# olsson-group/thermodynamic-interpolation

Hardware: AMD Instinct MI355X
Metric: integration-steps/sec (whole node) + drift rel-L2 vs CPU ref (higher is better)
Workload: dtype f32 state and accumulation; matrix products on fp16 MFMA with 2-way split fp32 operands (hi + lo halves, 3 products)

## Files before the change

### thermodynamic-interpolation_amd/csrc/api_painn.hip

```cpp
#include "rollout.hpp"

extern "C" {

ti_handle* ti_painn_create(const ti_painn_desc* d, const float* weights, size_t n_weights, const int32_t* edge_src,
                           const int32_t* edge_dst, const int32_t* edge_type, const int32_t* atom_ids, int device)
{
    ti_handle* out = nullptr;
    const int rc = guarded([&]() -> int {
        if (!d || !weights || !atom_ids) return fail(TI_E_ARG, "NULL argument");
        const int F = d->n_features, L = d->n_layers, A = d->n_atoms, E = d->n_edges;
        if (F != 32 && F != 64 && F != 128 && F != 256) return fail(TI_E_UNSUPPORTED, "n_features must be 32, 64, 128 or 256");
        if (L < 1) return fail(TI_E_ARG, "n_layers must be >= 1");
        if (A < 1 || A > 32) return fail(TI_E_UNSUPPORTED, "n_atoms must be in 1..32 (the reference caps it at n_types = 25)");
        if (E < 0 || (E > 0 && (!edge_src || !edge_dst || !edge_type))) return fail(TI_E_ARG, "edge arrays missing");
        if (d->variant < 0 || d->variant > 2) return fail(TI_E_ARG, "unknown variant");
        if (d->n_types < 1) return fail(TI_E_ARG, "n_types must be >= 1");
        if (d->precision != TI_PREC_F32 && d->precision != TI_PREC_F16X2 && d->precision != TI_PREC_F16) return fail(TI_E_ARG, "unknown precision");
        for (int k = 0; k < E; ++k)
            if (edge_src[k] < 0 || edge_src[k] >= A || edge_dst[k] < 0 || edge_dst[k] >= A || edge_type[k] < 0 || edge_type[k] > 3)
                return fail(TI_E_ARG, "edge index / type out of range");
        for (int a = 0; a < A; ++a) if (atom_ids[a] < 0 || atom_ids[a] >= d->n_types) return fail(TI_E_ARG, "atom id out of range");
        std::unique_ptr<ti_handle> h(new_handle(0, device));
        h->d = *d; h->NB = F / 32;
        h->nE = d->variant == TI_VARIANT_AMBIENT ? 4 : d->variant == TI_VARIANT_LATENT_MULTI ? 3 : 2;
// ... 223 lines not shown
            if (n_floats != N * F) return fail(TI_E_ARG, "size mismatch (s)");
            std::vector<float> ds(n_floats);
            HIP_CHECK(hipMemcpy(out, h->s.p, n_floats * sizeof(float), hipMemcpyDeviceToHost));
            HIP_CHECK(hipMemcpy(ds.data(), h->dsacc.p, n_floats * sizeof(float), hipMemcpyDeviceToHost));
            for (size_t i = 0; i < n_floats; ++i) out[i] += ds[i];
        } else if (what == 1) {
            if (n_floats != N * 3 * F) return fail(TI_E_ARG, "size mismatch (v)");
            std::vector<float> v(n_floats), dv(n_floats), cc(n_floats);
            HIP_CHECK(hipMemcpy(v.data(), h->v.p, n_floats * sizeof(float), hipMemcpyDeviceToHost));
            HIP_CHECK(hipMemcpy(dv.data(), h->dvacc.p, n_floats * sizeof(float), hipMemcpyDeviceToHost));
            HIP_CHECK(hipMemcpy(cc.data(), h->cacc.p, n_floats * sizeof(float), hipMemcpyDeviceToHost));
            for (size_t nd = 0; nd < N; ++nd)
                for (size_t f = 0; f < F; ++f)
                    for (int c = 0; c < 3; ++c) {
                        const int c1 = (c + 1) % 3, c2 = (c + 2) % 3;
                        auto at = [&](const std::vector<float>& a, int cc2) { return a[(nd * 3 + cc2) * F + f]; };
                        out[(nd * 3 + c) * F + f] = (at(v, c) + at(dv, c)) + (at(cc, c1) * at(v, c2) - at(cc, c2) * at(v, c1));
                    }
        } else if (what == 2) {
            if (n_floats != B * E * F) return fail(TI_E_ARG, "size mismatch (e)");
            const size_t RB = ti::EDGE_ROWS_PER_BLOCK, rows = (B + h->G - 1) / h->G * h->parts * h->nblk * RB * (h->active == 2 ? 2 : 1);
            std::vector<float> e(rows * F);
            HIP_CHECK(hipMemcpy(e.data(), h->e.p, e.size() * sizeof(float), hipMemcpyDeviceToHost));
            for (size_t m = 0; m < B; ++m)
                for (size_t k = 0; k < E; ++k)
                    std::memcpy(out + (m * E + h->perm[k]) * F, e.data() + edge_row_of(h, m, k) * F, F * sizeof(float));
        } else if (what >= 3 && what <= 5) {
            if (h->last_D != 1 || (size_t)h->last_VB != B) return fail(TI_E_ARG, "tangent taps need a preceding ti_painn_drift_jvp call");
            auto fetch = [&](const DevBuf<float>& b, size_t n) { std::vector<float> v(n); HIP_CHECK(hipMemcpy(v.data(), b.p, n * sizeof(float), hipMemcpyDeviceToHost)); return v; };
            if (what == 3) {
                if (n_floats != N * F) return fail(TI_E_ARG, "size mismatch (ts)");
                const auto ts = fetch(h->ts, n_floats), td = fetch(h->tdsacc, n_floats);
                for (size_t i = 0; i < n_floats; ++i) out[i] = ts[i] + td[i];
            } else if (what == 4) {
                if (n_floats != N * 3 * F) return fail(TI_E_ARG, "size mismatch (tv)");
                const auto v = fetch(h->v, n_floats), cc = fetch(h->cacc, n_floats);
                const auto tv = fetch(h->tv, n_floats), tdv = fetch(h->tdvacc, n_floats), tcc = fetch(h->tcacc, n_floats);
                for (size_t nd = 0; nd < N; ++nd)
                    for (size_t f = 0; f < F; ++f)
                        for (int c = 0; c < 3; ++c) {
                            const int c1 = (c + 1) % 3, c2 = (c + 2) % 3;
                            auto at = [&](const std::vector<float>& a, int cc2) { return a[(nd * 3 + cc2) * F + f]; };
                            out[(nd * 3 + c) * F + f] = (at(tv, c) + at(tdv, c)) + ((at(tcc, c1) * at(v, c2) + at(cc, c1) * at(tv, c2)) -
                                                                                     (at(tcc, c2) * at(v, c1) + at(cc, c2) * at(tv, c1)));
                        }
            } else {
                if (n_floats != B * E * F) return fail(TI_E_ARG, "size mismatch (te)");
                const size_t RB = ti::EDGE_ROWS_PER_BLOCK, rows = (B + h->G - 1) / h->G * h->parts * h->nblk * RB;
                const auto e = fetch(h->te, rows * F);
                for (size_t m = 0; m < B; ++m)
                    for (size_t k = 0; k < E; ++k)
                        std::memcpy(out + (m * E + h->perm[k]) * F, e.data() + edge_row_of(h, m, k) * F, F * sizeof(float));
            }
        } else return fail(TI_E_ARG, "unknown tap");
        return TI_OK;
    });
}

int ti_painn_set_template(ti_handle* h, int which)
{
    if (!h || h->kind != 0) return fail(TI_E_ARG, "not a painn handle");
    if (which != TI_TEMPLATE_AUTO && which != TI_TEMPLATE_THROUGHPUT && which != TI_TEMPLATE_LATENCY && which != TI_TEMPLATE_PAIR) return fail(TI_E_ARG, "unknown template");
    if (which == TI_TEMPLATE_LATENCY && h->n_tpl < 2) which = TI_TEMPLATE_THROUGHPUT;
    if (which == TI_TEMPLATE_PAIR && !h->has_pair) which = TI_TEMPLATE_THROUGHPUT;
    h->pinned_tpl = which;
    return TI_OK;
}

int ti_painn_template_for(ti_handle* h, int64_t B)
{
    if (!h || h->kind != 0) return fail(TI_E_ARG, "not a painn handle");
    if (h->has_pair && mask_blocks_pair(h) && pinned_template(h) == TI_TEMPLATE_PAIR)
        return fail(TI_E_UNSUPPORTED, "the pair layout is pinned, and the edge mask in force is not symmetric for every molecule");
    return template_for(h, B);
}

int ti_painn_set_edge_mask(ti_handle* h, const uint32_t* mask, int64_t B, int mem)
{
    if (mem != TI_MEM_HOST && mem != TI_MEM_DEVICE) return fail(TI_E_ARG, "unknown mem");
    if (mask && B < 1) return fail(TI_E_ARG, "B < 1");
    if (!h || h->kind != 0) return fail(TI_E_ARG, "not a painn handle");
    if (!mask) { clear_graph_state(h); return TI_OK; }
    return guarded([&]() -> int {
        set_device(h);
        const int A = h->d.n_atoms;
        std::vector<uint32_t> m((size_t)B * A);
        if (mem == TI_MEM_DEVICE) HIP_CHECK(hipMemcpy(m.data(), mask, m.size() * sizeof(uint32_t), hipMemcpyDeviceToHost));
        else std::memcpy(m.data(), mask, m.size() * sizeof(uint32_t));
        std::vector<int32_t> none; std::vector<uint8_t> no_types;
        return set_graph_state(h, m, none, no_types, B);
    });
}

int ti_painn_set_molecules(ti_handle* h, const int32_t* n_atoms, const uint32_t* mask, const uint8_t* pair_type, int64_t B, int mem)
{
    if (mem != TI_MEM_HOST && mem != TI_MEM_DEVICE) return fail(TI_E_ARG, "unknown mem");
    if (n_atoms && B < 1) return fail(TI_E_ARG, "B < 1");
    if (!h || h->kind != 0) return fail(TI_E_ARG, "not a painn handle");
    if (!n_atoms) { clear_graph_state(h); return TI_OK; }
    return guarded([&]() -> int {
        set_device(h);
        const int A = h->d.n_atoms;
        auto fetch = [&](void* dst, const void* src, size_t bytes) {
            if (mem == TI_MEM_DEVICE) HIP_CHECK(hipMemcpy(dst, src, bytes, hipMemcpyDeviceToHost));
            else std::memcpy(dst, src, bytes);
        };
// ... 18 lines not shown
```

### thermodynamic-interpolation_amd/csrc/painn_host.hip

```cpp
#include "ti_handle.hpp"

namespace ti {

void ensure_painn_ws(ti_handle* h, long long B)
{
    if (B <= h->cap) return;
    const size_t A = h->d.n_atoms, F = h->d.n_features, N = (size_t)B * A;
    h->x.alloc(N * 3); h->b1.alloc(N * 3); h->b2.alloc(N * 3); h->xt.alloc(N * 3);
    h->cond.alloc(std::max<size_t>(N * h->ncond, 1));
    const size_t se = h->d.precision == TI_PREC_F16 ? 2 : 1;
    h->s.alloc((N * F + se - 1) / se); h->P.alloc((N * F + se - 1) / se);
    h->v.alloc((N * 3 * F + se - 1) / se); h->dvacc.alloc(N * 3 * F); h->cacc.alloc(N * 3 * F); h->dsacc.alloc(N * F);
    h->e.alloc((edge_rows_for(h, B) * F + se - 1) / se);
    h->enc.alloc((edge_rows_for(h, B) * F + se - 1) / se); h->geo.alloc(edge_rows_for(h, B) * 4);
    h->divb.alloc(B); h->div2.alloc(B); h->dl.alloc(B); h->dlscaled.alloc(B);
    h->cap = B;
}

long long jvp_virtual_molecules(const ti_handle* h, long long B, int D) { return (B + h->G - 1) / h->G * D * h->G; }

size_t jvp_bytes_per_vm(const ti_handle* h)
{
    const size_t A = h->d.n_atoms, F = h->d.n_features;
    const size_t erows = ((size_t)h->parts * h->nblk * ti::EDGE_ROWS_PER_BLOCK + h->G - 1) / h->G;
// ... 158 lines not shown
        }
        if (h->nblk > 0) {
            EdgeParams p{};
            p.stream = h->S(h->st_edge[l]); p.nch = h->st_edge[l].nch; p.vecs = h->edge_vecs.p + (size_t)l * 21 * F;
            p.edge_emb = h->F(h->edge_emb); p.rows = h->rows.p; p.slotnode = h->slotnode.p; p.nslots = nullptr;
            p.nblk = h->nblk; p.G = h->G; p.parts = h->parts; p.A = A; p.max_slots = h->max_slots; p.B = B; p.n_groups = groups; p.length_scale = h->d.length_scale;
            p.x = x_dev; p.P = h->P.p; p.v = h->v.p; p.dsacc = h->dsacc.p; p.dvacc = h->dvacc.p; p.cacc = h->cacc.p; p.e = h->e.p; p.enc = h->enc.p; p.geo = h->geo.p;
            for (int i = 0; i < 6; ++i) p.wscale[i] = 1.0f;
            if (edge_one_chain(prec)) {
                p.stream = h->S(h->st_edge1[l]); p.nch = h->st_edge1[l].nch; p.vecs = h->edge_vecs1.p + (size_t)l * 21 * F;
                for (int i = 0; i < 6; ++i) p.wscale[i] = h->edge_scale[(size_t)l * 6 + i];
            }
            if (mrows) p.rows = mrows;
            Timed tm(h, TI_KERNEL_PAINN_EDGE);
#ifdef TI_STAMPS
            if (l == 2) p.stamps = stamps_arm(groups, st);
#endif
            if (h->active == 2) {
                HIP_CHECK(launch_pair(NB, l == 0, l == L - 1, prec, p, st, mrows != nullptr));
#ifdef TI_STAMPS
                stamps_dump(h, p.stamps, groups, st);
#endif
            } else {
                HIP_CHECK(launch_edge(NB, l == 0, l == L - 1, prec, p, st, mrows != nullptr));
#ifdef TI_STAMPS
                stamps_dump(h, p.stamps, groups, st);
#endif
            }
        }
        if (h->tap == 1 + 2 * l) return;
        if (jr) {
            {
                JvpNodeParams p{};
                p.stream = h->S(h->st_jvp_update[l]); p.nch = h->st_jvp_update[l].nch; p.vecs = h->upd_vecs.p + (size_t)l * 10 * F;
                p.N = N; p.s = h->s.p; p.v = h->v.p; p.dsacc = h->dsacc.p; p.dvacc = h->dvacc.p; p.cacc = h->cacc.p;
                p.ns = reinterpret_cast<float4*>(h->nodest.p);
                Timed tm(h, TI_KERNEL_PAINN_JVP_FILTER);
                HIP_CHECK(launch_jvp_node(NB, split, p, st));
            }
            JvpUpdateParams p{};
            p.stream = h->S(h->st_jvp_update[l]); p.nch = h->st_jvp_update[l].nch; p.vecs = h->upd_vecs.p + (size_t)l * 10 * F;
            p.N = VN; p.B = B; p.A = A; p.D = jr->D; p.G = h->G; p.has_next = l + 1 < L;
            p.v = h->v.p; p.cacc = h->cacc.p; p.ns = reinterpret_cast<const float4*>(h->nodest.p);
            p.ts = h->ts.p; p.tv = h->tv.p; p.tdsacc = h->tdsacc.p; p.tdvacc = h->tdvacc.p; p.tcacc = h->tcacc.p; p.tP = h->tP.p;
            p.zero_acc = !ft;
            Timed tm(h, TI_KERNEL_PAINN_JVP_UPDATE);
            HIP_CHECK(launch_jvp_update(NB, split, p, st));
        }
        {
            UpdateParams p{};
            p.stream = h->S(h->st_update[l]); p.nch = h->st_update[l].nch; p.vecs = h->upd_vecs.p + (size_t)l * 10 * F;
            p.N = N; p.s = h->s.p; p.v = h->v.p; p.dsacc = h->dsacc.p; p.dvacc = h->dvacc.p; p.cacc = h->cacc.p; p.P = h->P.p;
            p.first_layer = l == 0; p.zero_acc = !ft;
            const bool folded = h->nblk > 0 && h->active == 2 && l > 0 && pair_folds_cross(prec);
            Timed tm(h, TI_KERNEL_PAINN_UPDATE);
            HIP_CHECK(launch_update(NB, l + 1 < L, prec, p, st, folded));
        }
        if (h->tap == 2 + 2 * l) return;
    }
    if (jr) {
        JvpReadoutParams p{};
        p.stream = h->S(h->st_jvp_readout); p.nch = h->st_jvp_readout.nch; p.vecs = h->jvp_ro_vecs.p; p.b2_gate = h->b2_gate;
        p.N = VN; p.B = B; p.A = A; p.D = jr->D; p.G = h->G; p.s = h->s.p; p.v = h->v.p; p.ts = h->ts.p; p.tv = h->tv.p; p.tout = jr->tout;
        Timed tm(h, TI_KERNEL_PAINN_JVP_READOUT);
        HIP_CHECK(launch_jvp_readout(NB, split, p, st));
    }
    {
        ReadoutParams p{};
        p.stream = h->S(h->st_jvp_readout); p.nch = h->st_jvp_readout.nch; p.mlp = h->vec(h->readout);
        p.w2_gate = h->F(h->readout.W2 + F); p.b2_gate = h->b2_gate; p.Vr = h->F(h->Vr);
        p.N = N; p.s = h->s.p; p.v = h->v.p; p.out = out_dev;
        Timed tm(h, TI_KERNEL_PAINN_READOUT);
        HIP_CHECK(launch_readout(NB, prec, p, st));
    }
    if (nat) {
        HIP_CHECK(launch_zero_pads(out_dev, nat, B, 1, A, 3, st));
        if (jr && jr->D == 1) HIP_CHECK(launch_zero_pads(jr->tout, nat, B, 1, A, 3, st));
    }
}

void painn_drift_div_dev(ti_handle* h, const float* x_dev, float t, const float* cond_dev, long long B, float* out_dev, float* div_dev,
                         const float* tv)
{
    const int A = h->d.n_atoms, D = 3 * A;
    const long long chunk = jvp_chunk_molecules(h, D);
    for (long long b0 = 0; b0 < B; b0 += chunk) {
        const long long bc = std::min(chunk, B - b0);
        ensure_jvp_ws(h, bc, D);
        JvpRun jr{D, nullptr, h->tout.p};
        painn_drift_dev(h, x_dev + (size_t)b0 * A * 3, t, cond_dev ? cond_dev + (size_t)b0 * A * h->ncond : nullptr, bc,
                        out_dev + (size_t)b0 * A * 3, &jr, tv ? tv + b0 : nullptr, b0);
        if (h->ragged) HIP_CHECK(launch_div_reduce_ragged(h->tout.p, bc, D, h->G, h->natoms_dev.p + b0, div_dev + b0, h->stream));
        else HIP_CHECK(launch_div_reduce(h->tout.p, bc, D, h->G, div_dev + b0, h->stream));
    }
    h->last_B = std::min(chunk, B);
}

void painn_make_probes(ti_handle* h, long long B, int k, uint64_t seed, long long traj0)
{
    const int n3 = 3 * h->d.n_atoms;
    grow(h->probes, (size_t)B * k * n3);
    HIP_CHECK(launch_probes(h->probes.p, seed, traj0, B, k, n3, h->stream));
    if (h->ragged) HIP_CHECK(launch_zero_pads(h->probes.p, h->natoms_dev.p, B * k, k, h->d.n_atoms, 3, h->stream));
}

void painn_drift_div_est_dev(ti_handle* h, const float* x_dev, float t, const float* cond_dev, long long B, int k, float* out_dev,
// ... 57 lines not shown
```

### thermodynamic-interpolation_amd/csrc/painn_kernels.hip

```cpp
#include <hip/amd_detail/amd_hip_unsafe_atomics.h>

#include "dispatch.hpp"
#include "mfma_chain.hpp"
#include "ti_internal.hpp"

namespace ti {


struct UV {
    static constexpr int B0 = 0, G0 = 1, BE0 = 2, B1 = 3, G1 = 4, BE1 = 5, B2 = 6 , PB0 = 9, COUNT = 10;
};

__host__ __device__ constexpr int update_superchunk(int NB, bool H16) { return H16 && NB == 4 ? 4 : 2; }
__host__ __device__ constexpr int update_chunk4(int NB, bool H16) { return (H16 ? 128 : 256) * NB; }
template <int NBK, bool HAS_NEXT, int PREC, bool FOLDED = false>
__global__ __launch_bounds__(256, (NBK <= 8 ? 2 : 1)) void painn_update_kernel(const UpdateParams p)
{
    constexpr bool H16 = PREC == 2;
    constexpr int F = 16 * NBK, NB = (F + 31) / 32, WAVES = 4, T = 64 * WAVES, CH4 = update_chunk4(NB, H16);
    using A16 = r16::Act<NBK>;
    using OP = typename r16::OpSel<NBK, PREC>::type;
    extern __shared__ f32x4 lds[];
    const int lane = threadIdx.x & 63, wave = __builtin_amdgcn_readfirstlane(threadIdx.x >> 6), j = lane & 15, q = lane >> 4;
    constexpr int SC = update_superchunk(NB, H16);
    float* vec = reinterpret_cast<float*>(lds + 2 * SC * CH4);
    for (int i = threadIdx.x; i < UV::COUNT * F / 4; i += T)
        reinterpret_cast<f32x4*>(vec)[i] = reinterpret_cast<const f32x4*>(p.vecs)[i];
    PipeDMA<NB, T, SC, CH4> pipe;
    pipe.init(reinterpret_cast<const f32x4*>(p.stream), p.nch, lds, wave, lane);

    const long long node = ((long long)blockIdx.x * WAVES + wave) * 16 + j;
    const bool ok = node < p.N;
    const size_t nd = (size_t)(ok ? node : p.N - 1);
    const size_t vo = nd * 3 * F, so_ = nd * F;
    float* db = p.dvacc + nd * 3 * F;
    float* cb = p.cacc + nd * 3 * F;
    float* ab = p.dsacc + nd * F;

    A16 n2;
    {
        OP ve[3];
        float vsc[3];
        {
            A16 t[3];
#pragma unroll
            for (int nb = 0; nb < NBK; ++nb) {
                f32x4 vv[3], kk[3];
#pragma unroll
                for (int c = 0; c < 3; ++c) {
                    vv[c] = p.first_layer ? f32x4{0, 0, 0, 0} : r16::load_state<H16>(p.v, vo + c * F, nb, q);
                    kk[c] = p.first_layer || FOLDED ? f32x4{0, 0, 0, 0} : r16::load_block(cb + c * F, nb, q);
                }
#pragma unroll
                for (int c = 0; c < 3; ++c) {
                    const int c1 = (c + 1) % 3, c2 = (c + 2) % 3;
                    const f32x4 dd = r16::load_block(db + c * F, nb, q);
                    if (FOLDED) t[c].b[nb] = vv[c] + dd;
                    else t[c].b[nb] = (vv[c] + dd) + (kk[c1] * vv[c2] - kk[c2] * vv[c1]);
                    if (ok) r16::store_block(db + c * F, nb, q, t[c].b[nb]);
                }
            }
#pragma unroll
            for (int c = 0; c < 3; ++c) vsc[c] = ve[c].set_scaled(t[c]);
        }
#pragma unroll
        for (int nb = 0; nb < NBK; ++nb) n2.b[nb] = f32x4{0, 0, 0, 0};
#pragma unroll
        for (int ch = 0; ch < NB; ++ch) {
            const f32x4* wl = pipe.acquire();
#pragma unroll
            for (int c = 0; c < 3; ++c) {
                f32x4 a0 = {0, 0, 0, 0}, a1 = {0, 0, 0, 0};
                r16::gemm_bt(a0, a1, ve[c], wl, lane);
                a0 *= vsc[c]; a1 *= vsc[c];
                n2.b[2 * ch] += a0 * a0; n2.b[2 * ch + 1] += a1 * a1;
            }
            pipe.release();
        }
    }
    A16 snew;
    OP h2;
    {
        A16 t;
#pragma unroll
        for (int nb = 0; nb < NBK; ++nb) t.b[nb] = r16::load_block(vec + UV::B0 * F, nb, q);
        {
            OP nn;
            float nsc;
            {
                A16 u;
#pragma unroll
                for (int nb = 0; nb < NBK; ++nb)
#pragma unroll
                    for (int r = 0; r < 4; ++r) u.b[nb][r] = sqrtf(n2.b[nb][r]);
                nsc = nn.set_scaled(u);
            }
#pragma unroll
            for (int ch = 0; ch < NB; ++ch) {
                const f32x4* wl = pipe.acquire();
                f32x4 g0 = {0, 0, 0, 0}, g1 = {0, 0, 0, 0};
                r16::gemm_bt(g0, g1, nn, wl, lane);
                t.b[2 * ch] += g0 * nsc; t.b[2 * ch + 1] += g1 * nsc;
                pipe.release();
            }
        }
        {
            OP ss;
            float ssc;
#pragma unroll
            for (int nb = 0; nb < NBK; ++nb) snew.b[nb] = r16::load_state<H16>(p.s, so_, nb, q) + r16::load_block(ab, nb, q);
            ssc = ss.set_scaled(snew);
#pragma unroll
// ... 5 lines not shown
                pipe.release();
            }
        }
        r16::ln_silu(t, vec + UV::G0 * F, vec + UV::BE0 * F, q);
        OP h1;
        h1.set(t);
#pragma unroll
        for (int ch = 0; ch < NB; ++ch) {
            const f32x4* wl = pipe.acquire();
            f32x4 a0 = r16::load_block(vec + UV::B1 * F, 2 * ch, q), a1 = r16::load_block(vec + UV::B1 * F, 2 * ch + 1, q);
            r16::gemm_bt(a0, a1, h1, wl, lane);
            t.b[2 * ch] = a0; t.b[2 * ch + 1] = a1;
            pipe.release();
        }
        r16::ln_silu(t, vec + UV::G1 * F, vec + UV::BE1 * F, q);
        h2.set(t);
    }
#pragma unroll
    for (int ch = 0; ch < NB; ++ch) {
        const f32x4* wl = pipe.acquire();
        f32x4 q0 = r16::load_block(vec + (UV::B2 + 1) * F, 2 * ch, q), q1 = r16::load_block(vec + (UV::B2 + 1) * F, 2 * ch + 1, q);
        r16::gemm_bt(q0, q1, h2, wl, lane);
        pipe.release();
        wl = pipe.acquire();
        f32x4 a0 = r16::load_block(vec + (UV::B2 + 2) * F, 2 * ch, q), a1 = r16::load_block(vec + (UV::B2 + 2) * F, 2 * ch + 1, q);
        r16::gemm_bt(a0, a1, h2, wl, lane);
        pipe.release();
#pragma unroll
        for (int k = 0; k < 2; ++k) {
            const int nb = 2 * ch + k;
            f32x4 so = snew.b[nb];
            const f32x4 qq = k ? q1 : q0, aa = k ? a1 : a0;
#pragma unroll
            for (int r = 0; r < 4; ++r) {
                const float n = sqrtf(n2.b[nb][r]);
                so[r] = so[r] + ((n * n) * qq[r] + aa[r]);
            }
            snew.b[nb] = so;
            if (ok) {
                r16::store_state<H16>(p.s, so_, nb, q, so);
                if (p.zero_acc) r16::store_block(ab, nb, q, f32x4{0, 0, 0, 0});
            }
        }
    }
    A16 gg;
#pragma unroll
    for (int ch = 0; ch < NB; ++ch) {
        const f32x4* wl = pipe.acquire();
        f32x4 a0 = r16::load_block(vec + UV::B2 * F, 2 * ch, q), a1 = r16::load_block(vec + UV::B2 * F, 2 * ch + 1, q);
        r16::gemm_bt(a0, a1, h2, wl, lane);
        gg.b[2 * ch] = a0; gg.b[2 * ch + 1] = a1;
        pipe.release();
    }
#pragma unroll 1
    for (int c = 0; c < 3; ++c) {
        A16 t;
        r16::load_set(t, db + c * F, q);
        OP vc;
        const float usc = vc.set_scaled(t);
#pragma unroll
        for (int ch = 0; ch < NB; ++ch) {
            const f32x4* wl = pipe.acquire();
            f32x4 a0 = {0, 0, 0, 0}, a1 = {0, 0, 0, 0};
            r16::gemm_bt(a0, a1, vc, wl, lane);
            a0 *= usc; a1 *= usc;
            if (ok) {
                r16::store_state<H16>(p.v, vo + c * F, 2 * ch, q, t.b[2 * ch] + a0 * gg.b[2 * ch]);
                r16::store_state<H16>(p.v, vo + c * F, 2 * ch + 1, q, t.b[2 * ch + 1] + a1 * gg.b[2 * ch + 1]);
                if (p.zero_acc) {
                    r16::store_block(db + c * F, 2 * ch, q, f32x4{0, 0, 0, 0});
                    r16::store_block(db + c * F, 2 * ch + 1, q, f32x4{0, 0, 0, 0});
                    if (!FOLDED) {
                        r16::store_block(cb + c * F, 2 * ch, q, f32x4{0, 0, 0, 0});
                        r16::store_block(cb + c * F, 2 * ch + 1, q, f32x4{0, 0, 0, 0});
                    }
                }
            }
            pipe.release();
        }
    }
    if (HAS_NEXT) {
        OP sn;
        float psc;
        {
            psc = sn.set_scaled(snew);
        }
#pragma unroll
        for (int ch = 0; ch < NB; ++ch) {
            const f32x4* wl = pipe.acquire();
            f32x4 a0 = {0, 0, 0, 0}, a1 = {0, 0, 0, 0};
            r16::gemm_bt(a0, a1, sn, wl, lane);
            a0 = r16::load_block(vec + UV::PB0 * F, 2 * ch, q) + a0 * psc; a1 = r16::load_block(vec + UV::PB0 * F, 2 * ch + 1, q) + a1 * psc;
            pipe.release();
            if (ok) { r16::store_state<H16>(p.P, nd * F, 2 * ch, q, a0); r16::store_state<H16>(p.P, nd * F, 2 * ch + 1, q, a1); }
        }
    }
    pipe.drain();
}

template <int NBK, int NSEG, int PREC, bool TV = false>
__global__ __launch_bounds__(256, (NBK <= 8 ? 2 : 1)) void painn_embed16_kernel(const EmbedParams p)
{
    constexpr bool H16 = PREC == 2;
    constexpr int F = 16 * NBK, NB = (F + 31) / 32, WAVES = 4, T = 64 * WAVES, CH4 = update_chunk4(NB, H16);
    using A16 = r16::Act<NBK>;
    using OP = typename r16::OpSel<NBK, PREC>::type;
    extern __shared__ f32x4 lds[];
    const int lane = threadIdx.x & 63, wave = __builtin_amdgcn_readfirstlane(threadIdx.x >> 6), j = lane & 15, q = lane >> 4;
    PipeDMA<NB, T, 2, CH4> pipe;
    pipe.init(reinterpret_cast<const f32x4*>(p.stream), p.nch, lds, wave, lane);
    const long long node = ((long long)blockIdx.x * WAVES + wave) * 16 + j;
    const bool ok = node < p.N;
    const long long nd = ok ? node : p.N - 1;

    A16 acc;
#pragma unroll
    for (int nb = 0; nb < NBK; ++nb) acc.b[nb] = r16::load_block(p.mlp.b0, nb, q);
#pragma unroll
    for (int seg = 0; seg < NSEG; ++seg) {
        OP op;
        float sc = 1.0f;
        {
            A16 in;
            if (seg == 0) {
                r16::load_set(in, p.atom_emb + (size_t)p.atom_ids[nd % p.A] * F, q);
                sc = op.set_scaled(in);
            } else if (seg < NSEG - 1) {
                float u = p.cond[nd * p.ncond + (seg - 1)] - p.temp_mean;
                u = u / p.temp_range;
                r16::posenc_set(in, u / p.temp_length, q);
                op.set(in);
// ... 90 lines not shown
        }
        const float sinv = r16::pow2_inverse(ssc);
#pragma unroll
        for (int ch = 0; ch < NB; ++ch) {
            const f32x4* wl = pipe.acquire();
            f32x4 a0 = r16::load_block(p.mlp.b0, 2 * ch, q) * sinv, a1 = r16::load_block(p.mlp.b0, 2 * ch + 1, q) * sinv;
            r16::gemm_bt(a0, a1, sop, wl, lane);
            h1.b[2 * ch] = a0 * ssc; h1.b[2 * ch + 1] = a1 * ssc;
            pipe.release();
        }
    }
    r16::ln_silu(h1, p.mlp.g0, p.mlp.be0, q);
    A16 h2;
    {
        OP o1;
        o1.set(h1);
#pragma unroll
        for (int ch = 0; ch < NB; ++ch) {
            const f32x4* wl = pipe.acquire();
            f32x4 a0 = r16::load_block(p.mlp.b1, 2 * ch, q), a1 = r16::load_block(p.mlp.b1, 2 * ch + 1, q);
            r16::gemm_bt(a0, a1, o1, wl, lane);
            h2.b[2 * ch] = a0; h2.b[2 * ch + 1] = a1;
            pipe.release();
        }
    }
    pipe.drain();
    r16::ln_silu(h2, p.mlp.g1, p.mlp.be1, q);
    float gate = 0.f;
#pragma unroll
    for (int nb = 0; nb < NBK; ++nb) {
        const f32x4 w = r16::load_block(p.w2_gate, nb, q);
#pragma unroll
        for (int r = 0; r < 4; ++r) gate += h2.b[nb][r] * w[r];
    }
    gate = r16::xquarters(gate) + p.b2_gate;
#pragma unroll
    for (int c = 0; c < 3; ++c) {
        float vv = 0.f;
#pragma unroll
        for (int nb = 0; nb < NBK; ++nb) {
            const f32x4 x = r16::load_state<H16>(p.v, (nd * 3 + c) * F, nb, q), w = r16::load_block(p.Vr, nb, q);
#pragma unroll
            for (int r = 0; r < 4; ++r) vv += x[r] * w[r];
        }
        vv = r16::xquarters(vv);
        if (ok && q == 0) p.out[node * 3 + c] = vv * gate;
    }
}

static size_t update_lds_bytes(int NB, bool h16) { return 2 * update_superchunk(NB, h16) * (size_t)update_chunk4(NB, h16) * 16 + 10 * (size_t)32 * NB * 4; }
static size_t node16_lds_bytes(int NB, bool h16) { return 2 * 2 * (size_t)update_chunk4(NB, h16) * 16; }

enum NodeKernel { NODE_EMBED, NODE_UPDATE, NODE_READOUT };
constexpr bool node_build_exists(NodeKernel k, int PREC, int n, bool flag)
{
    return k == NODE_EMBED ? n >= 2 : k == NODE_UPDATE ? n <= 1 && (!flag || pair_folds_cross(PREC)) : n == 0 && !flag;
}
template <NodeKernel K, int NBK, int PREC, int N, bool FLAG>
constexpr auto node_kernel()
{
    if constexpr (K == NODE_EMBED) return painn_embed16_kernel<NBK, N, PREC, FLAG>;
    else if constexpr (K == NODE_UPDATE) return painn_update_kernel<NBK, N != 0, PREC, FLAG>;
    else return painn_readout16_kernel<NBK, PREC>;
}
template <NodeKernel K, class F>
static hipError_t with_node_builds(int NB, int prec, int n, int flag, F&& f)
{
    hipError_t e = hipSuccess;
    bool any = false;
    dispatch_int<1, 2, 4, 8>(NB, [&](auto bc) { dispatch_int<0, 1, 2>(prec, [&](auto pc) { dispatch_int<0, 1, 2, 3, 4>(n, [&](auto nc) { dispatch_bool(flag, [&](auto fc) {
        constexpr int nb = decltype(bc)::value, PREC = decltype(pc)::value, N = decltype(nc)::value;
        constexpr bool FLAG = decltype(fc)::value;
        if constexpr (node_build_exists(K, PREC, N, FLAG)) {
            any = true;
            if (e == hipSuccess) e = f(node_kernel<K, 2 * nb, PREC, N, FLAG>(), K == NODE_UPDATE ? update_lds_bytes(nb, PREC == 2) : node16_lds_bytes(nb, PREC == 2));
        }
    }); }); }); });
    return any ? e : hipErrorInvalidValue;
}
template <NodeKernel K>
static hipError_t configure_node(int NB)
{
    return with_node_builds<K>(NB, EVERY, EVERY, EVERY, [](auto kernel, size_t lds) { return set_lds(kernel, lds); });
}
template <NodeKernel K, class P>
static hipError_t launch_node(int NB, int prec, int n, bool flag, const P& p, hipStream_t st)
{
    return with_node_builds<K>(NB, prec, n, flag, [&](auto kernel, size_t lds) {
        hipLaunchKernelGGL(kernel, dim3((unsigned)((p.N + 63) / 64)), dim3(256), lds, st, p);
        return hipGetLastError();
    });
}

template <class F>
static hipError_t with_message_units(int NB, int masked, F&& f)
{
    hipError_t e = hipSuccess;
    const bool any = dispatch_int<1, 2, 4, 8>(NB, [&](auto bc) { dispatch_bool(masked, [&](auto mc) { if (e == hipSuccess) e = f(bc, mc); }); });
    return any ? e : hipErrorInvalidValue;
}

hipError_t configure_painn_kernels(int NB)
{
    hipError_t e;
    if ((e = configure_node<NODE_EMBED>(NB)) != hipSuccess) return e;
    if ((e = configure_node<NODE_UPDATE>(NB)) != hipSuccess) return e;
    if ((e = configure_node<NODE_READOUT>(NB)) != hipSuccess) return e;
    return with_message_units(NB, EVERY, [](auto bc, auto mc) {
        constexpr int nb = decltype(bc)::value;
        constexpr bool MASK = decltype(mc)::value;
        hipError_t e = configure_edge_unit<nb, MASK>();
        if constexpr (pair_build_exists(nb, 4, TI_PREC_F32)) { if (e == hipSuccess) e = configure_pair_unit<nb, MASK>(); }
        return e;
    });
}

hipError_t launch_embed(int NB, int nseg, int prec, const EmbedParams& p, hipStream_t st)
{
    return launch_node<NODE_EMBED>(NB, prec, nseg, p.tv != nullptr, p, st);
}
hipError_t launch_update(int NB, bool has_next, int prec, const UpdateParams& p, hipStream_t st, bool folded)
{
    return launch_node<NODE_UPDATE>(NB, prec, has_next, folded, p, st);
}
hipError_t launch_readout(int NB, int prec, const ReadoutParams& p, hipStream_t st) { return launch_node<NODE_READOUT>(NB, prec, 0, false, p, st); }

hipError_t launch_edge(int NB, bool first, bool last, int prec, const EdgeParams& p, hipStream_t st, bool masked)
{
    return with_message_units(NB, masked, [&](auto bc, auto mc) { return launch_edge_unit<decltype(bc)::value, decltype(mc)::value>(first, last, prec, p, st); });
}
hipError_t launch_pair(int NB, bool first, bool last, int prec, const EdgeParams& p, hipStream_t st, bool masked)
{
    return with_message_units(NB, masked, [&](auto bc, auto mc) {
        constexpr int nb = decltype(bc)::value;
        if constexpr (pair_build_exists(nb, 4, TI_PREC_F32)) return launch_pair_unit<nb, decltype(mc)::value>(first, last, prec, p, st);
        else return hipErrorInvalidValue;
    });
}

}
```

### thermodynamic-interpolation_amd/csrc/painn_pack.hip

```cpp
#include "pair_template.hpp"
#include "ti_handle.hpp"

namespace ti {

void pack_chunk16(std::vector<float>& dst, const float* W, int ld, int n_rows, int row0, int col0, int NBK)
{
    const size_t base = dst.size();
    dst.resize(base + (size_t)2 * NBK * 64 * 4);
    for (int blk = 0; blk < 2; ++blk)
        for (int nbi = 0; nbi < NBK; ++nbi)
            for (int l = 0; l < 64; ++l)
                for (int r = 0; r < 4; ++r) {
                    const int row = row0 + 16 * blk + (l & 15), col = col0 + 16 * nbi + 4 * (l >> 4) + r;
                    dst[base + ((size_t)(blk * NBK + nbi) * 64 + l) * 4 + r] = row < n_rows ? W[(size_t)row * ld + col] : 0.f;
                }
}

void pack_chunk16_split(std::vector<float>& dst, const float* W, int ld, int n_rows, int row0, int col0, int NBK)
{
    const size_t base = dst.size();
    dst.resize(base + (size_t)2 * NBK * 64 * 4);
    _Float16* out = reinterpret_cast<_Float16*>(dst.data() + base);
    const int KS = NBK / 2;
    for (int blk = 0; blk < 2; ++blk)
// ... 66 lines not shown
static int pack_part(const ti_handle* h, const int32_t* dst, int count, int k0, int k1, std::vector<int>& pos)
{
    constexpr int RB = ti::EDGE_ROWS_PER_BLOCK;
    const int per = k1 - k0;
    pos.assign((size_t)count * per, 0);
    int row = 0, nslot = 0, last_key = -1;
    for (int m = 0; m < count; ++m)
        for (int k = k0; k < k1; ++k) {
            const int key = m * 256 + dst[h->perm[k]];
            if (row % RB == 0) { nslot = 0; last_key = -1; }
            if (key != last_key) {
                if (nslot == ti::EDGE_MAX_SLOTS) { row = (row + RB - 1) / RB * RB; nslot = 0; }
                ++nslot; last_key = key;
            }
            pos[(size_t)m * per + (k - k0)] = row++;
        }
    return (row + RB - 1) / RB;
}

static int fill_part(const ti_handle* h, const int32_t* src, const int32_t* dst, const int32_t* etype, int count, int k0, int k1, int nblk,
                     const std::vector<int>& pos, uint32_t* rw, int32_t* sn)
{
    constexpr int RB = ti::EDGE_ROWS_PER_BLOCK;
    const int per = k1 - k0;
    for (int i = 0; i < nblk * RB; ++i) { rw[i] = (uint32_t)63 << 18; sn[i] = -1; }
    std::vector<int> nslot(std::max(nblk, 1), 0), last_key(std::max(nblk, 1), -1);
    std::vector<char> touched((size_t)count * 256, 0);
    int most = 0;
    for (int m = 0; m < count; ++m)
        for (int kk = 0; kk < per; ++kk) {
            const int r = pos[(size_t)m * per + kk], blk = r / RB, k = h->perm[k0 + kk];
            const int key = m * 256 + dst[k];
            if (key != last_key[blk]) {
                const int32_t first = (h->first_touch && !touched[key]) ? ti::SLOT_FIRST_TOUCH : 0;
                touched[key] = 1;
                sn[(size_t)blk * RB + nslot[blk]] = first | (m << 8) | dst[k]; ++nslot[blk]; last_key[blk] = key;
            }
            most = std::max(most, nslot[blk]);
            rw[r] = 1u | ((uint32_t)m << 1) | ((uint32_t)src[k] << 6) | ((uint32_t)dst[k] << 11) | ((uint32_t)etype[k] << 16) |
                    ((uint32_t)(nslot[blk] - 1) << 18);
        }
    return most;
}

void build_templates(ti_handle* h, const int32_t* src, const int32_t* dst, const int32_t* etype)
{
    const int A = h->d.n_atoms, E = h->d.n_edges;
    constexpr int RB = ti::EDGE_ROWS_PER_BLOCK;
    {
        std::vector<char> has_in(A, 0);
        for (int k = 0; k < E; ++k) has_in[dst[k]] = 1;
        h->first_touch = E > 0 && std::all_of(has_in.begin(), has_in.end(), [](char c) { return c != 0; });
        if (const char* z = std::getenv("TI_ZERO_ACC")) if (z[0] == '1') h->first_touch = false;
    }
    h->perm.resize(E);
    for (int k = 0; k < E; ++k) h->perm[k] = k;
    std::stable_sort(h->perm.begin(), h->perm.end(), [&](int a, int b) {
        return dst[a] != dst[b] ? dst[a] < dst[b] : src[a] < src[b];
    });
    {
        int bestG = 1; double bestW = 2.0;
        std::vector<int> pos;
        for (int G = 1; G <= 8 && E > 0; ++G) {
            const int rows = G * E, padded = pack_part(h, dst, G, 0, E, pos) * RB;
            const double waste = double(padded - rows) / padded;
            if (waste < bestW - 1e-12) { bestW = waste; bestG = G; }
            if (waste <= 0.02) { bestG = G; break; }
        }
        ti_handle::Tpl& T = h->tpl[0];
        T.G = bestG; T.P = 1;
        T.nblk = E > 0 ? pack_part(h, dst, bestG, 0, E, T.pos) : 0;
        T.part_of.assign(E, 0); T.part_start.assign(1, 0); T.part_len.assign(1, E);
        std::vector<uint32_t> rw((size_t)std::max(T.nblk, 1) * RB); std::vector<int32_t> sn(rw.size());
        T.max_slots = fill_part(h, src, dst, etype, bestG, 0, E, T.nblk, T.pos, rw.data(), sn.data());
        if (T.nblk == 0) { rw[0] = (uint32_t)63 << 18; sn[0] = -1; }
        T.rows.upload(rw); T.slotnode.upload(sn); T.rows_h = rw;
    }
    h->n_tpl = 1;
    if (E >= 2 * RB) {
        std::vector<int> first_of(A + 1, E);
        for (int k = E - 1; k >= 0; --k) first_of[dst[h->perm[k]]] = k;
        for (int a = A - 1; a >= 0; --a) first_of[a] = std::min(first_of[a], first_of[a + 1]);
        std::vector<int> pos;
        int bestP = 1, best_nblk = pack_part(h, dst, 1, 0, E, pos); std::vector<int> best_cut{0, E};
        for (int P = 2; P <= 8; ++P) {
            std::vector<int> cut{0};
            for (int q = 1; q < P; ++q) {
                const int want = (int)((long long)E * q / P);
                int bk = cut.back();
                for (int a = 0; a <= A; ++a) if (first_of[a] > cut.back() && std::abs(first_of[a] - want) < std::abs(bk - want)) bk = first_of[a];
                if (bk <= cut.back()) { cut.clear(); break; }
                cut.push_back(bk);
            }
            if (cut.empty() || cut.back() >= E) continue;
            cut.push_back(E);
            int nblk = 0;
            for (int q = 0; q < P; ++q) nblk = std::max(nblk, pack_part(h, dst, 1, cut[q], cut[q + 1], pos));
            if (double(P * nblk * RB - E) / (P * nblk * RB) <= 0.15) { bestP = P; best_nblk = nblk; best_cut = cut; }
        }
        if (bestP * h->tpl[0].G > 1) {
            ti_handle::Tpl& T = h->tpl[1];
            T.G = 1; T.P = bestP; T.nblk = best_nblk; T.max_slots = 0;
            T.part_start.assign(best_cut.begin(), best_cut.end() - 1);
            T.part_of.resize(E); T.part_len.resize(bestP); T.pos.assign(E, 0);
            for (int q = 0; q < bestP; ++q) for (int k = best_cut[q]; k < best_cut[q + 1]; ++k) T.part_of[k] = q;
            std::vector<uint32_t> rw((size_t)bestP * best_nblk * RB); std::vector<int32_t> sn(rw.size());
// ... 266 lines not shown
```

### thermodynamic-interpolation_amd/csrc/ti_handle.hpp

```cpp
#pragma once
#include <algorithm>
#include <array>
#include <climits>
#include <cmath>
#include <cstdio>
#include <cstdlib>
#include <cstring>
#include <map>
#include <memory>
#include <stdexcept>
#include <string>
#include <utility>
#include <vector>

#include "ti_internal.hpp"

namespace ti {

int fail(int code, const std::string& msg);

struct HipError : std::runtime_error { using std::runtime_error::runtime_error; };
struct Unsupported : std::runtime_error { using std::runtime_error::runtime_error; };
#define HIP_CHECK(expr) do { hipError_t e__ = (expr); if (e__ != hipSuccess) \
    throw HipError(std::string(#expr) + ": " + hipGetErrorString(e__)); } while (0)

constexpr const char* MSG_NO_FP16_TANGENT = "the fp16 storage mode has no divergence / tangent path (use f32 or f16x2)";
constexpr const char* MSG_TRAJ_OBSERVER = "TI_SCHEME_DOPRI5_TRAJ writes its rows per trajectory inside a kernel: detach the observer (ti_obs_set_observer)";
constexpr const char* MSG_TAP_ENTRIES = "debug taps apply to ti_painn_drift / ti_painn_drift_jvp only";
constexpr const char* MSG_EM_DLOGP = "dlogp is defined for a deterministic flow: EM needs eps = 0";

struct MlpOff { size_t W0, b0, g0, be0, W1, b1, g1, be1, W2, b2; int f_in, f_h, f_out; };

template <typename T>
struct DevBuf {
    T* p = nullptr; size_t n = 0;
    void alloc(size_t count) { release(); if (count) { HIP_CHECK(hipMalloc((void**)&p, count * sizeof(T))); n = count; } }
    void upload(const std::vector<T>& h) { alloc(h.size()); if (n) HIP_CHECK(hipMemcpy(p, h.data(), n * sizeof(T), hipMemcpyHostToDevice)); }
    void release() { if (p) { (void)hipFree(p); p = nullptr; n = 0; } }
    ~DevBuf() { release(); }
};

template <typename T>
void grow(DevBuf<T>& b, size_t n) { if (b.n < n) b.alloc(n); }

struct Stream { size_t off4; int nch; };

}

using namespace ti;

struct ti_handle {
    int kind = 0;
    int device = 0;
    hipStream_t own_stream = nullptr, stream = nullptr;
    hipEvent_t wait_ev = nullptr;
    bool prof = false;
    std::vector<std::pair<hipEvent_t, hipEvent_t>> ev[TI_KERNEL_COUNT];
    DevBuf<float> flat, packed;
    DevBuf<int> nanflag;
    long long cap = 0;

    ti_painn_desc d{};
    int NB = 0, nE = 0, ncond = 0, G = 1, nblk = 0;
    MlpOff embed{}, readout{}; std::vector<MlpOff> phi, w, upd; std::vector<size_t> U, V;
    size_t edge_emb = 0, atom_emb = 0, Vr = 0; float b2_gate = 0.f;
    Stream st_embed16{}; std::vector<Stream> st_edge, st_edge1, st_update;
    struct Tpl {
        int G = 1, P = 1, nblk = 0;
        DevBuf<uint32_t> rows; DevBuf<int32_t> slotnode;
        std::vector<uint32_t> rows_h;
        std::vector<int> part_of, part_start, part_len;
        std::vector<int> pos;
        int max_slots = 0;
    } tpl[3];
    bool has_pair = false; std::vector<int> pair_pos; double pair_fill = 0.0;
    int n_tpl = 1, active = 0, parts = 1, max_slots = 0, pinned_tpl = TI_TEMPLATE_AUTO;
    bool first_touch = false;
    std::vector<uint32_t> emask; long long emask_B = 0; bool emask_sym = true;
    DevBuf<uint32_t> mrows[3]; bool mrows_ok[3] = {false, false, false};
    std::vector<int32_t> natoms; std::vector<uint8_t> ptype; bool ragged = false; long long n_real = 0;
    DevBuf<int32_t> natoms_dev; DevBuf<float> xpark, cpark, dpark;
    struct { const uint32_t* p = nullptr; } rows; struct { const int32_t* p = nullptr; } slotnode;
    DevBuf<int32_t> atom_ids;
    std::vector<int> perm;
    std::vector<int32_t> esrc, edst;
    DevBuf<float> x, cond, s, P, v, dsacc, dvacc, cacc, e, enc, geo, b1, b2, xt, edge_vecs, edge_vecs1, upd_vecs;
    std::vector<float> edge_scale;
    int tap = -1; long long last_B = 0;
    std::vector<Stream> st_jvp_update, st_jvp_phi; Stream st_jvp_readout{}; std::vector<int> jvp_phi_pad;
    DevBuf<float> jvp_ro_vecs, ts, tP, tv, tdsacc, tdvacc, tcacc, te, tout, wq, phist, nodest, divb, dl, dlscaled, div2;
    long long jvp_cap = 0, last_VB = 0; int last_D = 1;
    DevBuf<float> probes;
    DevBuf<float> rk_ws; DevBuf<double> rk_red;
    DevBuf<TrajCtl> rk_ctl; DevBuf<float> rk_tv, rk_path, rk_dpath; DevBuf<int> rk_status; DevBuf<double> rk_grid;
    std::vector<int64_t> traj_accepted, traj_rejected;

    ti_adw_desc ad{};
    size_t a_be_vecs = 0, a_net_vecs = 0;
    float a_be_b_out = 0.f, a_b_out = 0.f;
    int a_dim = 1;
    Stream st_be{}, st_net{};
    DevBuf<float> ax, ab1, ab2, axt, aemb_u, abeta0_u, abeta1_u, adl, ad1, ad2; DevBuf<int32_t> aidx;
    DevBuf<float> abeta0_r, abeta1_r, aemb_r, atv;
    DevBuf<float> af_b0, af_b1, af_tv, af_emb, af_path, af_dl; DevBuf<AdwFusedStep> af_steps;

    struct ObsSet { int K = 0; bool has_ref = false, has_sel = false; DevBuf<int32_t> desc, sel; DevBuf<float> ref; } obs[2];
    int obs_every = 0, obs_mem = TI_MEM_HOST; float* obs_out = nullptr;
    DevBuf<float> obs_x, obs_cv, obs_val, obs_logw, obs_w; DevBuf<double> obs_red, obs_part;

    ~ti_handle()
    {
        for (auto& v2 : ev) for (auto& pr : v2) { (void)hipEventDestroy(pr.first); (void)hipEventDestroy(pr.second); }
        if (wait_ev) (void)hipEventDestroy(wait_ev);
        if (own_stream) (void)hipStreamDestroy(own_stream);
    }
    const float* F(size_t off) const { return flat.p + off; }
    const float4* S(const Stream& s2) const { return reinterpret_cast<const float4*>(packed.p) + s2.off4; }
    MlpVec vec(const MlpOff& m) const { return MlpVec{F(m.b0), F(m.g0), F(m.be0), F(m.b1), F(m.g1), F(m.be1), F(m.b2)}; }
};

namespace ti {

struct Timed {
    ti_handle* h; int slot; hipEvent_t a = nullptr, b = nullptr;
    Timed(ti_handle* h_, int slot_) : h(h_), slot(slot_)
    {
        if (!h->prof) return;
        HIP_CHECK(hipEventCreate(&a)); HIP_CHECK(hipEventCreate(&b));
        HIP_CHECK(hipEventRecord(a, h->stream));
    }
// ... 100 lines not shown
```

### thermodynamic-interpolation_amd/csrc/ti_internal.hpp

```cpp
#pragma once
#include <hip/hip_runtime.h>
#include <stdint.h>

#include <algorithm>
#include <string>
#include <vector>

#include "../../include/ti_hip.h"

namespace ti {

constexpr int32_t SLOT_FIRST_TOUCH = 1 << 30;
__host__ __device__ inline int slot_mol(int32_t sn) { return (sn >> 8) & 0x3fffff; }
constexpr int ROW_VALID = 1;
constexpr int EDGE_ROWS_PER_BLOCK = 16;
constexpr int EDGE_MAX_SLOTS = 4;
__host__ __device__ inline int row_mol(uint32_t w) { return (w >> 1) & 31; }
__host__ __device__ inline int row_src(uint32_t w) { return (w >> 6) & 31; }
__host__ __device__ inline int row_dst(uint32_t w) { return (w >> 11) & 31; }
__host__ __device__ inline int row_type(uint32_t w) { return (w >> 16) & 3; }
__host__ __device__ inline int row_slot(uint32_t w) { return (w >> 18) & 63; }

constexpr int PAIR_MAX_G = 8;
__host__ __device__ inline int prow_molI(uint32_t w) { return (w >> 1) & 7; }
__host__ __device__ inline int prow_atomI(uint32_t w) { return (w >> 4) & 31; }
__host__ __device__ inline int prow_molJ(uint32_t w) { return (w >> 9) & 7; }
__host__ __device__ inline int prow_atomJ(uint32_t w) { return (w >> 12) & 31; }
__host__ __device__ inline int prow_type(uint32_t w) { return (w >> 17) & 3; }

struct MlpVec {
    const float *b0, *g0, *be0, *b1, *g1, *be1, *b2;
};

struct EdgeParams {
    const float4* stream; int nch;
    const float* vecs;
    const float* edge_emb;
    const uint32_t* rows; const int32_t* slotnode; const int32_t* nslots;
    int nblk, G, parts, A;
    int max_slots;
    long long B, n_groups;
    float length_scale;
    const float* x;
    const float* P;
    const float* v;
    float* dsacc;
    float* dvacc;
    float* cacc;
    float* e;
    float* enc;
    float wscale[6];
    float* geo;
    unsigned long long* stamps;
};

struct EmbedParams {
    const float4* stream; int nch;
    MlpVec mlp; const float* pb0;
    const float* atom_emb; const int32_t* atom_ids; const float* cond;
    int ncond, A; long long N;
    float t, temp_length, time_length, temp_mean, temp_range;
    const float* tv;
    float* s; float* P;
};

struct UpdateParams {
    const float4* stream; int nch;
    const float* vecs;
    long long N;
    float *s, *v, *dsacc, *dvacc, *cacc, *P;
    int first_layer;
    int zero_acc;
};

struct ReadoutParams {
    const float4* stream; int nch;
    MlpVec mlp; const float* w2_gate; float b2_gate; const float* Vr;
    long long N;
    const float *s, *v; float* out;
};

hipError_t launch_embed(int NB, int nseg, int prec, const EmbedParams& p, hipStream_t st);
hipError_t launch_edge(int NB, bool first, bool last, int prec, const EdgeParams& p, hipStream_t st, bool masked = false);
__host__ __device__ constexpr bool edge_one_chain(int prec) { return prec == TI_PREC_F16X2; }
hipError_t launch_pair(int NB, bool first, bool last, int prec, const EdgeParams& p, hipStream_t st, bool masked = false);
__host__ __device__ constexpr bool pair_build_exists(int NB, int WAVES, int PREC)
{
    return (NB == 1 || NB == 2 || NB == 4) && (PREC == TI_PREC_F32 ? WAVES == 4 : PREC == TI_PREC_F16X2 && (WAVES == 4 || WAVES == 8));
}
__host__ __device__ constexpr bool pair_folds_cross(int prec) { return prec == TI_PREC_F16X2; }
hipError_t launch_update(int NB, bool has_next, int prec, const UpdateParams& p, hipStream_t st, bool folded = false);
hipError_t launch_readout(int NB, int prec, const ReadoutParams& p, hipStream_t st);
hipError_t configure_painn_kernels(int NB);
template <int NB, bool MASK> hipError_t launch_edge_unit(bool first, bool last, int prec, const EdgeParams& p, hipStream_t st);
template <int NB, bool MASK> hipError_t configure_edge_unit();
template <int NB, bool MASK> hipError_t launch_pair_unit(bool first, bool last, int prec, const EdgeParams& p, hipStream_t st);
template <int NB, bool MASK> hipError_t configure_pair_unit();

struct JvpFilterParams {
    const float4* stream; int nch; const float* vecs; const float* edge_emb;
    const uint32_t* rows;
    int nblk, G, parts, A, first, last;
    long long B, n_groups;
    float length_scale;
    const float *x, *P, *e;
    float4* wq;
    float4* st;
};
struct JvpEdgeParams {
    const float4* stream; int nch, pad; const float* vecs; const float* edge_emb;
    const uint32_t* rows; const int32_t* slotnode;
    int nblk, G, parts, A, D, first, last;
    long long B, n_groups;
    const float *x, *xdot;
    const float *P, *v, *e;
    const float4 *wq, *st;
    const float *tP, *tv;
    float *te, *tdsacc, *tdvacc, *tcacc;
};
struct JvpNodeParams {
    const float4* stream; int nch; const float* vecs;
    long long N;
    const float *s, *v, *dsacc, *dvacc, *cacc;
    float4* ns;
};
// ... 150 lines not shown
```

Before: 455,100.

## Keep formed vector rows in registers in update kernel instead of parking to dvacc

```diff
diff --git a/thermodynamic-interpolation_amd/csrc/api_painn.hip b/thermodynamic-interpolation_amd/csrc/api_painn.hip
--- a/thermodynamic-interpolation_amd/csrc/api_painn.hip
+++ b/thermodynamic-interpolation_amd/csrc/api_painn.hip
@@ -299,6 +299,10 @@
                     for (size_t k = 0; k < E; ++k)
                         std::memcpy(out + (m * E + h->perm[k]) * F, e.data() + edge_row_of(h, m, k) * F, F * sizeof(float));
             }
+        } else if (what == 6 || what == 7) {
+            if (h->d.precision == TI_PREC_F16) return fail(TI_E_UNSUPPORTED, "raw reads are of fp32 state; not available in the fp16 storage mode");
+            if (n_floats != N * 3 * F) return fail(TI_E_ARG, "size mismatch (raw v / dvacc)");
+            HIP_CHECK(hipMemcpy(out, what == 6 ? h->v.p : h->dvacc.p, n_floats * sizeof(float), hipMemcpyDeviceToHost));
         } else return fail(TI_E_ARG, "unknown tap");
         return TI_OK;
     });
diff --git a/thermodynamic-interpolation_amd/csrc/painn_host.hip b/thermodynamic-interpolation_amd/csrc/painn_host.hip
--- a/thermodynamic-interpolation_amd/csrc/painn_host.hip
+++ b/thermodynamic-interpolation_amd/csrc/painn_host.hip
@@ -234,6 +234,7 @@
             p.stream = h->S(h->st_update[l]); p.nch = h->st_update[l].nch; p.vecs = h->upd_vecs.p + (size_t)l * 10 * F;
             p.N = N; p.s = h->s.p; p.v = h->v.p; p.dsacc = h->dsacc.p; p.dvacc = h->dvacc.p; p.cacc = h->cacc.p; p.P = h->P.p;
             p.first_layer = l == 0; p.zero_acc = !ft;
+            p.no_park = ft && !jr && h->update_keeps_rows;
             const bool folded = h->nblk > 0 && h->active == 2 && l > 0 && pair_folds_cross(prec);
             Timed tm(h, TI_KERNEL_PAINN_UPDATE);
             HIP_CHECK(launch_update(NB, l + 1 < L, prec, p, st, folded));
diff --git a/thermodynamic-interpolation_amd/csrc/painn_kernels.hip b/thermodynamic-interpolation_amd/csrc/painn_kernels.hip
--- a/thermodynamic-interpolation_amd/csrc/painn_kernels.hip
+++ b/thermodynamic-interpolation_amd/csrc/painn_kernels.hip
@@ -13,9 +13,10 @@
 
 __host__ __device__ constexpr int update_superchunk(int NB, bool H16) { return H16 && NB == 4 ? 4 : 2; }
 __host__ __device__ constexpr int update_chunk4(int NB, bool H16) { return (H16 ? 128 : 256) * NB; }
-template <int NBK, bool HAS_NEXT, int PREC, bool FOLDED = false>
+template <int NBK, bool HAS_NEXT, int PREC, bool FOLDED = false, int KEEP = 0>
 __global__ __launch_bounds__(256, (NBK <= 8 ? 2 : 1)) void painn_update_kernel(const UpdateParams p)
 {
+    static_assert(KEEP == 0 || KEEP == 3 || FOLDED, "a row that is formed again is v + dvacc: no cross term");
     constexpr bool H16 = PREC == 2;
     constexpr int F = 16 * NBK, NB = (F + 31) / 32, WAVES = 4, T = 64 * WAVES, CH4 = update_chunk4(NB, H16);
     using A16 = r16::Act<NBK>;
@@ -37,12 +38,13 @@
     float* cb = p.cacc + nd * 3 * F;
     float* ab = p.dsacc + nd * F;
 
+    const bool park = !KEEP && !(p.no_park && p.first_layer);
     A16 n2;
+    A16 t[3];
     {
         OP ve[3];
         float vsc[3];
         {
-            A16 t[3];
 #pragma unroll
             for (int nb = 0; nb < NBK; ++nb) {
                 f32x4 vv[3], kk[3];
@@ -57,7 +59,7 @@
                     const f32x4 dd = r16::load_block(db + c * F, nb, q);
                     if (FOLDED) t[c].b[nb] = vv[c] + dd;
                     else t[c].b[nb] = (vv[c] + dd) + (kk[c1] * vv[c2] - kk[c2] * vv[c1]);
-                    if (ok) r16::store_block(db + c * F, nb, q, t[c].b[nb]);
+                    if (park && ok) r16::store_block(db + c * F, nb, q, t[c].b[nb]);
                 }
             }
 #pragma unroll
@@ -169,10 +171,7 @@
         gg.b[2 * ch] = a0; gg.b[2 * ch + 1] = a1;
         pipe.release();
     }
-#pragma unroll 1
-    for (int c = 0; c < 3; ++c) {
-        A16 t;
-        r16::load_set(t, db + c * F, q);
+    auto component = [&](const int c, const A16& t) __attribute__((always_inline)) {
         OP vc;
         const float usc = vc.set_scaled(t);
 #pragma unroll
@@ -194,6 +193,30 @@
                 }
             }
             pipe.release();
+        }
+    };
+    if constexpr (KEEP) {
+#pragma unroll
+        for (int c = 0; c < 3; ++c) {
+            if (c < KEEP) component(c, t[c]);
+            else {
+                A16 tc;
+#pragma unroll
+                for (int nb = 0; nb < NBK; ++nb)
+                    tc.b[nb] = r16::load_state<H16>(p.v, vo + c * F, nb, q) + r16::load_block(db + c * F, nb, q);
+                component(c, tc);
+            }
+        }
+    } else {
+#pragma unroll 1
+        for (int c = 0; c < 3; ++c) {
+            A16 tc;
+            if (park) r16::load_set(tc, db + c * F, q);
+            else {
+#pragma unroll
+                for (int nb = 0; nb < NBK; ++nb) tc.b[nb] = f32x4{0, 0, 0, 0} + r16::load_block(db + c * F, nb, q);
+            }
+            component(c, tc);
         }
     }
     if (HAS_NEXT) {
@@ -390,15 +413,18 @@
 static size_t node16_lds_bytes(int NB, bool h16) { return 2 * 2 * (size_t)update_chunk4(NB, h16) * 16; }
 
 enum NodeKernel { NODE_EMBED, NODE_UPDATE, NODE_READOUT };
-constexpr bool node_build_exists(NodeKernel k, int PREC, int n, bool flag)
-{
-    return k == NODE_EMBED ? n >= 2 : k == NODE_UPDATE ? n <= 1 && (!flag || pair_folds_cross(PREC)) : n == 0 && !flag;
+constexpr int update_keep(int NBK, int PREC) { return !pair_folds_cross(PREC) ? 0 : NBK <= 4 ? 3 : NBK == 8 ? 2 : 0; }
+constexpr bool node_build_exists(NodeKernel k, int NBK, int PREC, int n, bool flag)
+{
+    return k == NODE_EMBED ? n >= 2
+         : k == NODE_UPDATE ? (n <= 1 || (n <= 3 && flag && update_keep(NBK, PREC) > 0)) && (!flag || pair_folds_cross(PREC))
+                            : n == 0 && !flag;
 }
 template <NodeKernel K, int NBK, int PREC, int N, bool FLAG>
 constexpr auto node_kernel()
 {
     if constexpr (K == NODE_EMBED) return painn_embed16_kernel<NBK, N, PREC, FLAG>;
-    else if constexpr (K == NODE_UPDATE) return painn_update_kernel<NBK, N != 0, PREC, FLAG>;
+    else if constexpr (K == NODE_UPDATE) return painn_update_kernel<NBK, (N & 1) != 0, PREC, FLAG, (N >= 2 ? update_keep(NBK, PREC) : 0)>;
     else return painn_readout16_kernel<NBK, PREC>;
 }
 template <NodeKernel K, class F>
@@ -409,7 +435,7 @@
     dispatch_int<1, 2, 4, 8>(NB, [&](auto bc) { dispatch_int<0, 1, 2>(prec, [&](auto pc) { dispatch_int<0, 1, 2, 3, 4>(n, [&](auto nc) { dispatch_bool(flag, [&](auto fc) {
         constexpr int nb = decltype(bc)::value, PREC = decltype(pc)::value, N = decltype(nc)::value;
         constexpr bool FLAG = decltype(fc)::value;
-        if constexpr (node_build_exists(K, PREC, N, FLAG)) {
+        if constexpr (node_build_exists(K, 2 * nb, PREC, N, FLAG)) {
             any = true;
             if (e == hipSuccess) e = f(node_kernel<K, 2 * nb, PREC, N, FLAG>(), K == NODE_UPDATE ? update_lds_bytes(nb, PREC == 2) : node16_lds_bytes(nb, PREC == 2));
         }
@@ -459,7 +485,8 @@
 }
 hipError_t launch_update(int NB, bool has_next, int prec, const UpdateParams& p, hipStream_t st, bool folded)
 {
-    return launch_node<NODE_UPDATE>(NB, prec, has_next, folded, p, st);
+    const bool keep = p.no_park && folded && update_keep(2 * NB, prec) > 0;
+    return launch_node<NODE_UPDATE>(NB, prec, (int)has_next + 2 * (int)keep, folded, p, st);
 }
 hipError_t launch_readout(int NB, int prec, const ReadoutParams& p, hipStream_t st) { return launch_node<NODE_READOUT>(NB, prec, 0, false, p, st); }
 
diff --git a/thermodynamic-interpolation_amd/csrc/painn_pack.hip b/thermodynamic-interpolation_amd/csrc/painn_pack.hip
--- a/thermodynamic-interpolation_amd/csrc/painn_pack.hip
+++ b/thermodynamic-interpolation_amd/csrc/painn_pack.hip
@@ -142,6 +142,7 @@
         for (int k = 0; k < E; ++k) has_in[dst[k]] = 1;
         h->first_touch = E > 0 && std::all_of(has_in.begin(), has_in.end(), [](char c) { return c != 0; });
         if (const char* z = std::getenv("TI_ZERO_ACC")) if (z[0] == '1') h->first_touch = false;
+        if (const char* z = std::getenv("TI_UPDATE_PARK")) if (z[0] == '1') h->update_keeps_rows = false;
     }
     h->perm.resize(E);
     for (int k = 0; k < E; ++k) h->perm[k] = k;
diff --git a/thermodynamic-interpolation_amd/csrc/ti_handle.hpp b/thermodynamic-interpolation_amd/csrc/ti_handle.hpp
--- a/thermodynamic-interpolation_amd/csrc/ti_handle.hpp
+++ b/thermodynamic-interpolation_amd/csrc/ti_handle.hpp
@@ -76,6 +76,7 @@
     bool has_pair = false; std::vector<int> pair_pos; double pair_fill = 0.0;
     int n_tpl = 1, active = 0, parts = 1, max_slots = 0, pinned_tpl = TI_TEMPLATE_AUTO;
     bool first_touch = false;
+    bool update_keeps_rows = true;
     std::vector<uint32_t> emask; long long emask_B = 0; bool emask_sym = true;
     DevBuf<uint32_t> mrows[3]; bool mrows_ok[3] = {false, false, false};
     std::vector<int32_t> natoms; std::vector<uint8_t> ptype; bool ragged = false; long long n_real = 0;
diff --git a/thermodynamic-interpolation_amd/csrc/ti_internal.hpp b/thermodynamic-interpolation_amd/csrc/ti_internal.hpp
--- a/thermodynamic-interpolation_amd/csrc/ti_internal.hpp
+++ b/thermodynamic-interpolation_amd/csrc/ti_internal.hpp
@@ -71,6 +71,7 @@
     float *s, *v, *dsacc, *dvacc, *cacc, *P;
     int first_layer;
     int zero_acc;
+    int no_park;
 };
 
 struct ReadoutParams {
```

After: 461,600, median of 6. +1.4%, better.
